# karthik86248/BANG-Billion-Scale-ANN

Measured on AMD Instinct MI355X. Metric: queries/sec, 10K-query batch; SHAPE-ONLY index, L=152, 201 iterations/query (cap-bound), recall n/a; recall-gated: config.recall_gated_* (structured index, 10-recall@10 >= 0.9). A shape-only batch is heavier per query than real data at recall 0.9, higher is better.
Workload: dtype f32

## Files before the change

bang-billion-scale-ann_amd/csrc/bang_search.hip:

```cpp

#include <hip/hip_runtime.h>
#include <type_traits>
#include <utility>
#include <stdint.h>
#include <stdlib.h>
#include <algorithm>

#include "bang_c.h"
#include "bang_internal.h"
#include "bang_device.h"
#include "bang_worklist.h"

struct SearchArgs;
template <class T>
__device__ __forceinline__ T karg_at(size_t off) {
  const char __attribute__((address_space(4)))* ka = (const char __attribute__((address_space(4)))*)__builtin_amdgcn_kernarg_segment_ptr();
  asm volatile("" : "+s"(ka));
  return *(const T __attribute__((address_space(4)))*)(ka + off);
}
__device__ __forceinline__ uint64_t scalar_load_u64(uint64_t tab, uint32_t idx) {
  uint64_t v;
  const uint64_t a = tab + 8ull * idx;
  const uint64_t at = ((uint64_t)uni((uint32_t)(a >> 32)) << 32) | uni((uint32_t)a);
  asm volatile("s_load_dwordx2 %0, %1, 0x0\n\ts_waitcnt lgkmcnt(0)" : "=s"(v) : "s"(at) : "memory");
  return v;
}
#define KARG(field) karg_at<decltype(bang_search_params::field)>(offsetof(SearchArgs, p) + offsetof(bang_search_params, field))
#define KARGP(type, field) ((type GAS*)(uintptr_t)KARG(field))

struct IterArgs {
  const uint8_t* d_codes; uint32_t n_nodes, prio;
  uint32_t* d_cand_ids; const uint8_t* d_graph; uint64_t entry_len;
  uint32_t vec_bytes, row_layout, n_rows_hbm, n_slices;
  const uint32_t* d_rows_hbm; const uint64_t* d_row_slices;
  uint32_t slice_rows, summ_iters;
  uint32_t* d_bloom; uint32_t cap_iter, pad1;
};
enum { IA_CODES = 0, IA_N_NODES = 2, IA_PRIO = 3, IA_CAND_IDS = 4, IA_GRAPH = 6, IA_ENTRY_LEN = 8, IA_VEC_BYTES = 10, IA_ROW_LAYOUT = 11, IA_N_ROWS_HBM = 12,
       IA_N_SLICES = 13, IA_ROWS_HBM = 14, IA_ROW_SLICES = 16, IA_SLICE_ROWS = 18, IA_SUMM_ITERS = 19, IA_BLOOM = 20, IA_CAP_ITER = 22, IA_DWORDS = 24 };
static_assert(sizeof(IterArgs) == 4 * IA_DWORDS && offsetof(IterArgs, d_cand_ids) == 4 * IA_CAND_IDS && offsetof(IterArgs, vec_bytes) == 4 * IA_VEC_BYTES &&
              offsetof(IterArgs, d_rows_hbm) == 4 * IA_ROWS_HBM && offsetof(IterArgs, slice_rows) == 4 * IA_SLICE_ROWS && offsetof(IterArgs, d_bloom) == 4 * IA_BLOOM && offsetof(IterArgs, cap_iter) == 4 * IA_CAP_ITER,
              "IterArgs dword map");
struct SearchArgs {
  bang_search_params p;
  IterArgs iter __attribute__((aligned(16)));
  uint32_t lds_piv_floats;
  uint32_t wave_words;
  uint32_t wl_words;
  uint32_t nctx;
  uint32_t gs;
};

__host__ __device__ constexpr bool search_coop(int ndw, bool host_paced) { return ndw >= 12 && (!host_paced || ndw >= 16); }
__host__ __device__ constexpr bool search_has_spec(int ndw) { return ndw == 18 || ndw == 19; }
__host__ __device__ constexpr int search_maxt(int ndw, bool host_paced);
__host__ __device__ constexpr uint32_t search_scratch_words(int ndw, bool host_paced);

__host__ __device__ inline uint32_t search_wl_words(uint32_t L) { return (2u * L + (L + 3u) / 4u + 3u) & ~3u; }
__host__ __device__ inline uint32_t search_wave_words(uint32_t L, uint32_t nctx, int ndw, bool host_paced) {
  return nctx * search_wl_words(L) + search_scratch_words(ndw, host_paced) + (nctx == 2 ? 32u : 0u);
}

template <int SLOTS>
__device__ __forceinline__ void filter_commit(uint32_t* tbl, int lane, bool& pa, uint32_t ia, uint32_t ba, uint32_t wa, bool& pb,
                                              uint32_t ib, uint32_t bb, uint32_t wb, bool& st_a, uint32_t& out_a, bool& st_b,
                                              uint32_t& out_b) {
  const uint32_t tag_a = (ia << 7) | ((uint32_t)lane << 1), tag_b = (ib << 7) | ((uint32_t)lane << 1) | 1u;
#pragma unroll
  for (int r = 0; r < 3; ++r) {
    if (__ballot(pa || pb) == 0) break;
    const uint32_t mul = r == 0 ? 0x9E37u : r == 1 ? 0x85EBu : 0xC2B3u;
    const uint32_t sa = ((ia * mul) >> 9) & (uint32_t)(SLOTS - 1), sb = ((ib * mul) >> 9) & (uint32_t)(SLOTS - 1);
    if (pa) tbl[sa] = tag_a;
    if (pb) tbl[sb] = tag_b;
    wave_sync();
    const uint32_t ra = tbl[sa], rb = tbl[sb];
    const bool own_a = pa && ra == tag_a, own_b = pb && rb == tag_b;
    const bool same_a = pa && !own_a && (ra >> 7) == ia, same_b = pb && !own_b && (rb >> 7) == ib;
    wave_sync();
    uint32_t va = ba, vb = bb;
    if (__ballot(same_a || same_b)) {
      if (own_a) tbl[sa] = ba;
      if (own_b) tbl[sb] = bb;
      wave_sync();
      if (same_a) (void)__hip_atomic_fetch_or(&tbl[sa], ba, __ATOMIC_RELAXED, __HIP_MEMORY_SCOPE_WAVEFRONT);
      if (same_b) (void)__hip_atomic_fetch_or(&tbl[sb], bb, __ATOMIC_RELAXED, __HIP_MEMORY_SCOPE_WAVEFRONT);
      wave_sync();
      if (own_a) va = tbl[sa];
      if (own_b) vb = tbl[sb];
      wave_sync();
    }
    if (own_a && (wa | va) != wa) { st_a = true; out_a = wa | va; }
    if (own_b && (wb | vb) != wb) { st_b = true; out_b = wb | vb; }
    pa = pa && !(own_a || same_a);
    pb = pb && !(own_b || same_b);
  }
}

#ifndef BANG_FILTER_SUMMARY
#define BANG_FILTER_SUMMARY 1
#endif
template <int SUMM_REGS>
struct FilterSummary {
  uint32_t s[SUMM_REGS];
  __device__ __forceinline__ void clear() {
#pragma unroll
    for (int r = 0; r < SUMM_REGS; ++r) s[r] = 0u;
  }
  static __device__ __forceinline__ uint32_t pos_of(uint32_t w) { const uint32_t p = w >> 6; return p >= 32u * SUMM_REGS ? p - 32u * SUMM_REGS : p; }
  __device__ __forceinline__ bool test(uint32_t w) const {
    const uint32_t p = pos_of(w);
    const int src = (int)((w & 63u) << 2);
    uint32_t v = 0;
#pragma unroll
    for (int r = 0; r < SUMM_REGS; ++r) {
      const uint32_t t = (uint32_t)__builtin_amdgcn_ds_bpermute(src, (int)s[r]);
      v = ((p >> 5) == (uint32_t)r) ? t : v;
    }
    return ((v >> (p & 31u)) & 1u) != 0u;
  }
  template <int RP>
  __device__ __forceinline__ void set(uint32_t* tbl , int lane, bool ha, uint32_t wa, bool hb, uint32_t wb,
                                      bool hc, uint32_t wc0, uint32_t wc1) {
    const uint32_t pa = pos_of(wa), pb = pos_of(wb), pc0 = pos_of(wc0), pc1 = pos_of(wc1);
#pragma unroll
    for (int pass = 0; pass < (SUMM_REGS + RP - 1) / RP; ++pass) {
      if (RP == 2 ? 2 * pass >= SUMM_REGS : 4 * pass >= SUMM_REGS) break;
      const bool ia = ha && (pa >> 5) / RP == (uint32_t)pass, ib = hb && (pb >> 5) / RP == (uint32_t)pass;
      const bool ic0 = hc && (pc0 >> 5) / RP == (uint32_t)pass, ic1 = hc && (pc1 >> 5) / RP == (uint32_t)pass;
      if (__ballot(ia || ib || ic0 || ic1) == 0) continue;
      if (RP == 2) *(uint2*)(tbl + 2 * lane) = make_uint2(0u, 0u);
      else *(uint4*)(tbl + 4 * lane) = make_uint4(0u, 0u, 0u, 0u);
      wave_sync();
      if (ia) (void)__hip_atomic_fetch_or(&tbl[(wa & 63u) * RP + ((pa >> 5) % RP)], 1u << (pa & 31u), __ATOMIC_RELAXED, __HIP_MEMORY_SCOPE_WAVEFRONT);
      if (ib) (void)__hip_atomic_fetch_or(&tbl[(wb & 63u) * RP + ((pb >> 5) % RP)], 1u << (pb & 31u), __ATOMIC_RELAXED, __HIP_MEMORY_SCOPE_WAVEFRONT);
      if (ic0) (void)__hip_atomic_fetch_or(&tbl[(wc0 & 63u) * RP + ((pc0 >> 5) % RP)], 1u << (pc0 & 31u), __ATOMIC_RELAXED, __HIP_MEMORY_SCOPE_WAVEFRONT);
      if (ic1) (void)__hip_atomic_fetch_or(&tbl[(wc1 & 63u) * RP + ((pc1 >> 5) % RP)], 1u << (pc1 & 31u), __ATOMIC_RELAXED, __HIP_MEMORY_SCOPE_WAVEFRONT);
      wave_sync();
      if (RP == 2) {
        const uint2 v = *(const uint2*)(tbl + 2 * lane);
        s[2 * pass] |= v.x;
        if (2 * pass + 1 < SUMM_REGS) s[2 * pass + 1] |= v.y;
      } else {
        const uint4 v = *(const uint4*)(tbl + 4 * lane);
        s[4 * pass] |= v.x;
        if (4 * pass + 1 < SUMM_REGS) s[4 * pass + 1] |= v.y;
        if (4 * pass + 2 < SUMM_REGS) s[4 * pass + 2] |= v.z;
        if (4 * pass + 3 < SUMM_REGS) s[4 * pass + 3] |= v.w;
      }
      wave_sync();
    }
  }
};

__device__ __forceinline__ void group_barrier(uint32_t* bar, uint32_t n, int lane) {
  asm volatile("s_waitcnt lgkmcnt(0)" ::: "memory");
  if (n > 1 && lane == 0) {
    const uint32_t gen = __hip_atomic_load(&bar[1], __ATOMIC_RELAXED, __HIP_MEMORY_SCOPE_WORKGROUP);
    const uint32_t arrived = __hip_atomic_fetch_add(&bar[0], 1u, __ATOMIC_RELAXED, __HIP_MEMORY_SCOPE_WORKGROUP) + 1u;
    if (arrived == n) {
      __hip_atomic_store(&bar[0], 0u, __ATOMIC_RELAXED, __HIP_MEMORY_SCOPE_WORKGROUP);
      asm volatile("s_waitcnt lgkmcnt(0)" ::: "memory");
      __hip_atomic_store(&bar[1], gen + 1u, __ATOMIC_RELAXED, __HIP_MEMORY_SCOPE_WORKGROUP);
    } else {
      while (__hip_atomic_load(&bar[1], __ATOMIC_RELAXED, __HIP_MEMORY_SCOPE_WORKGROUP) == gen) __builtin_amdgcn_s_sleep(1);
    }
  }
  asm volatile("s_waitcnt lgkmcnt(0)" ::: "memory");
  wave_sync();
}

#define SRCH_GO_STOP 0xFFFFFFFFu
#define SRCH_FIN 0xFFFFFFFFu
#define SRCH_CTX_WORDS 16u

#ifndef BANG_LONG_MAXT
#define BANG_LONG_MAXT 768
#endif

__host__ __device__ constexpr int search_maxt(int ndw, bool host_paced) { return (search_coop(ndw, host_paced) && ndw >= 16) ? (host_paced ? 768 : BANG_LONG_MAXT) : 1024; }
__host__ __device__ constexpr uint32_t search_scratch_words(int ndw, bool host_paced) {
  return search_coop(ndw, host_paced) ? ((ndw >= 16 && search_maxt(ndw, host_paced) >= 1024) ? 144u : 256u) : 144u;
}

template <int PSZ, int NDW, bool ALIGNED, int NHI, bool HOST, bool SPEC>
__global__ __launch_bounds__(search_maxt(NDW, HOST)) void search_kernel(const SearchArgs a) {
  extern __shared__ __attribute__((aligned(16))) float lds[];
  const bang_search_params& p = a.p;
  float* piv_lds = lds;
  {
    const float4* src = (const float4*)p.d_pivots_packed;
    float4* dst = (float4*)piv_lds;
    const uint32_t n4 = a.lds_piv_floats >> 2;
    for (uint32_t i0 = threadIdx.x; i0 < n4; i0 += blockDim.x * 8) {
      float4 v[8];
#pragma unroll
      for (int j = 0; j < 8; ++j) {
        const uint32_t i = i0 + (uint32_t)j * blockDim.x;
        v[j] = src[i < n4 ? i : n4 - 1];
      }
#pragma unroll
      for (int j = 0; j < 8; ++j) {
        const uint32_t i = i0 + (uint32_t)j * blockDim.x;
        if (i < n4) dst[i] = v[j];
      }
    }
  }
  const int lane0 = lane_id();
  int lane = lane0;
  const uint32_t wave = uni(threadIdx.x >> 6);
  const uint32_t nwaves = blockDim.x >> 6;
  uint32_t iav;
  {
    const char __attribute__((address_space(4)))* ka = (const char __attribute__((address_space(4)))*)__builtin_amdgcn_kernarg_segment_ptr();
    iav = ((const uint32_t __attribute__((address_space(4)))*)(ka + offsetof(SearchArgs, iter)))[lane0 < IA_DWORDS ? lane0 : 0];
  }
#define IA_FRESH() asm volatile("" : "+v"(iav))
#define IA32(k) ((uint32_t)__builtin_amdgcn_readlane((int)iav, (k)))
#define IA64(k) (((uint64_t)IA32((k) + 1) << 32) | (uint64_t)IA32(k))
#define IAPTR(type, k) ((type GAS*)IA64(k))
  const uint32_t nctx = HOST ? a.nctx : 1u;
  const uint32_t L = p.L, medoid = p.medoid;
  const unsigned long long go_timeout = p.go_timeout_ticks ? p.go_timeout_ticks : BANG_KERNEL_GO_TIMEOUT_TICKS;
  uint32_t* wbase = (uint32_t*)(lds + a.lds_piv_floats) + (size_t)wave * a.wave_words;
  uint32_t* scratch = wbase + (size_t)nctx * a.wl_words;
  uint32_t* park = scratch + search_scratch_words(NDW, HOST);
  const uint32_t gs = HOST ? a.gs : nwaves;
  const uint32_t grp_in_wg = HOST ? wave / gs : 0u;
  const uint32_t gw0 = grp_in_wg * gs;
  const uint32_t gsize = (nwaves - gw0) < gs ? (nwaves - gw0) : gs;
  const uint32_t gslot = wave - gw0;
  const uint32_t ngrp = HOST ? (nwaves + gs - 1) / gs : 1u;
  uint32_t* wg_lds = (uint32_t*)(lds + a.lds_piv_floats) + (size_t)nwaves * a.wave_words + (size_t)grp_in_wg * 128;
  if (HOST && gslot == 0) { wg_lds[lane] = 0u; wg_lds[64 + lane] = 0u; }
  if (HOST && nctx == 2 && lane < (int)(2 * SRCH_CTX_WORDS)) park[lane] = 0u;
  __syncthreads();
  if (p.d_ktime && threadIdx.x == 0) p.d_ktime[2 * blockIdx.x] = __builtin_amdgcn_s_memrealtime();

  float* sd = (float*)scratch;
  uint32_t* ti = scratch;
  float* td = (float*)(scratch + 72);
  uint32_t* sc = scratch + 72;
  uint32_t* tbl = scratch;
  const uint32_t total_waves = gridDim.x * nwaves;
  const uint32_t gw = blockIdx.x * nwaves + wave;
  const uint32_t cand_stride = L + BANG_EXTRA_ITERS;
  constexpr int SB = (NDW >= 18) ? 6 : 0;
  constexpr bool EARLY_ROWS = !HOST;
  constexpr bool COOP = search_coop(NDW, HOST);
  constexpr uint32_t SCR = search_scratch_words(NDW, HOST);
  static_assert(!SPEC || !HOST, "the speculative row request belongs to the self-paced form");

  const uint32_t code_stride = p.code_stride ? p.code_stride : p.m;

  bool active = false, exhausted = false;
  uint32_t q = 0, iter = 0, w_n = 0, cc = 0, mark = 0, evals = 0, fetched = 0;
  uint32_t cnt_in = 0, x0 = 0, x1 = 0;
  bool have_row = false;
  bool self_row = false;
  WlHead head;
  head.found = false; head.idx = 0; head.id = 0; head.d = 0.0f; head.tail = 0.0f;
  constexpr int QW = NDW * 4 * PSZ;
  constexpr bool QC16 = !HOST && ((NDW == 18 && NHI != 0) || NDW == 19);
  constexpr int NV = QC16 ? (QW + 15) / 16 : (QW + 63) / 64;
  typedef typename std::conditional<QC16, QcRow16<NV>, QcRegs<NV>>::type Qc;
  Qc qc;
#pragma unroll
  for (int r = 0; r < NV; ++r) qc.v[r] = 0.0f;
  auto load_qc = [&](uint32_t qq) {
    const float* src = p.d_qc + (size_t)qq * QW;
#pragma unroll
    for (int r = 0; r < NV; ++r) {
      const uint32_t i = QC16 ? (uint32_t)r * 16u + ((uint32_t)lane & 15u) : (uint32_t)r * 64u + (uint32_t)lane;
      qc.v[r] = src[i < (uint32_t)QW ? i : 0u];
    }
  };
  constexpr bool SUMM = (BANG_FILTER_SUMMARY != 0) && (!HOST || search_maxt(NDW, HOST) < 1024);
  FilterSummary<6> summ;
  summ.clear();
  uint32_t probes_skipped = 0;
  uint32_t started = 0;
  uint32_t dead_mask = 0;
  uint32_t rounds0 = 0, rounds1 = 0;
  uint32_t tick = 0;

  unsigned long long pf_poll = 0, pf_front = 0, pf_pub = 0, pf_back = 0, pf_n = 0, pf_t = 0;
  const bool prof = HOST && p.d_prof != nullptr && wave == 0;
#define PF_STAMP(acc) do { if (prof) { const unsigned long long t_ = __builtin_amdgcn_s_memrealtime(); acc += t_ - pf_t; pf_t = t_; } } while (0)
  if (prof) pf_t = __builtin_amdgcn_s_memrealtime();

#ifdef BANG_SEARCH_PHASE_PROF
  unsigned long long ph_acc[12] = {0, 0, 0, 0, 0, 0, 0, 0, 0, 0, 0, 0}, ph_t = __builtin_amdgcn_s_memrealtime(), ph_n = 0;
#define PH(k) do { if (wave == 0) { const unsigned long long t_ = __builtin_amdgcn_s_memrealtime(); ph_acc[k] += t_ - ph_t; ph_t = t_; } } while (0)
#else
#define PH(k) do {} while (0)
#endif

#define LANE_FRESH() do { if (BANG_LONG_MAXT >= 1024) { lane = lane0; asm volatile("" : "+v"(lane)); } } while (0)
  for (uint32_t half = 0;; ++half) {
    LANE_FRESH();
    const uint32_t c = HOST ? (nctx == 2 ? (half & 1u) : 0u) : 0u;
    if (HOST) {
      if (dead_mask == (nctx == 2 ? 3u : 1u)) break;
      if ((dead_mask >> c) & 1u) continue;
    }
    const uint32_t round = HOST ? (c ? rounds1 : rounds0) + 1u : 0u;
    const uint32_t grp = HOST ? (blockIdx.x * ngrp + grp_in_wg) * nctx + c : 0u;
    WaveLds s;
    s.wd = (float*)(wbase + (size_t)c * a.wl_words); s.wi = wbase + (size_t)c * a.wl_words + L; s.wv = (uint8_t*)(wbase + (size_t)c * a.wl_words + 2 * L);
    s.sd = sd; s.ti = ti; s.td = td;
    if (HOST) {
      if (nctx == 2) {
        const uint32_t* pk = park + c * SRCH_CTX_WORDS;
        active = uni(pk[0]) != 0u; q = uni(pk[1]); iter = uni(pk[2]); w_n = uni(pk[3]); cc = uni(pk[4]); mark = uni(pk[5]);
        evals = uni(pk[6]); fetched = uni(pk[7]);
        have_row = uni(pk[8]) != 0u;
        head.found = uni(pk[9]) != 0u; head.idx = uni(pk[10]); head.id = uni(pk[11]);
        head.d = __uint_as_float(uni(pk[12])); head.tail = __uint_as_float(uni(pk[13]));
        if (active) load_qc(q);
      }
      if (round > 1) {
        if (gslot == 0 && lane == 0) {
          const uint32_t* go = p.d_ctl + (size_t)grp * 16;
          uint32_t v = __hip_atomic_load(go, __ATOMIC_RELAXED, __HIP_MEMORY_SCOPE_SYSTEM);
          const unsigned long long t0 = __builtin_amdgcn_s_memrealtime();
          while (v < round - 1u) {
            __builtin_amdgcn_s_sleep(4);
            v = __hip_atomic_load(go, __ATOMIC_RELAXED, __HIP_MEMORY_SCOPE_SYSTEM);
            if (__builtin_amdgcn_s_memrealtime() - t0 > go_timeout) {
              v = SRCH_GO_STOP;
              if (p.d_abort) *p.d_abort = 1u;
              break;
            }
          }
          wg_lds[0] = v;
          __builtin_amdgcn_fence(__ATOMIC_ACQUIRE, "agent");
          asm volatile("s_waitcnt vmcnt(0)" ::: "memory");
        }
        group_barrier(wg_lds + 120, gsize, lane);
        PF_STAMP(pf_poll);
        if (wg_lds[0] == SRCH_GO_STOP) break;
        if (active && have_row && !self_row) {
          const uint32_t cw = p.d_ctl[(size_t)grp * 16 + 1 + (gslot >> 2)];
          cnt_in = (cw >> (8 * (gslot & 3u))) & 0xFFu;
          x0 = p.d_rows[((size_t)grp * 16 + gslot) * 64 + lane];
        }
      }
    }

    if (!active && !exhausted) {
      if (!((started >> c) & 1u)) q = c * total_waves + gw;
      else {
        uint32_t t = 0;
        if (lane == 0) t = __hip_atomic_fetch_add(KARGP(uint32_t, d_next_query), 1u, __ATOMIC_RELAXED, __HIP_MEMORY_SCOPE_AGENT);
        q = nctx * total_waves + uni(t);
      }
      started |= 1u << c;
      if (q < KARG(Q)) {
        active = true;
        w_n = 0; cc = 1; mark = 0x01010101u;
        evals = 0; fetched = 0; iter = 1;
        if (SUMM) { summ.clear(); probes_skipped = 0; }
        if (lane == 0) KARGP(uint32_t, d_cand_ids)[(size_t)q * cand_stride] = medoid;
        load_qc(q);
        { const uint32_t GAS* seed = KARGP(const uint32_t, d_seed); cnt_in = seed[0]; x0 = seed[1 + lane]; x1 = seed[65]; }
        have_row = true;
        self_row = false;
      } else exhausted = true;
    }
    if (!HOST && !active) break;

    uint32_t n = 0, sid0 = 0, sid1 = 0, parent = 0;
    constexpr bool SET_LATE = !HOST;
    bool sl_a = false, sl_b = false;
    uint32_t sl_ua = 0, sl_ub = 0;
    float d0 = BIG_DIST, d1 = BIG_DIST;
    bool found = false;
    const bool first = (iter == 1);
    if (active) {
      uint32_t ci = have_row ? uni(cnt_in) : 0u;
      if (((!HOST && p.row_layout) || (HOST && self_row)) && !first && have_row)
        ci = (uint32_t)__popcll(__ballot(x0 != 0xFFFFFFFFu));
      PH(0);
      {
        const uint32_t cap = p.R + (first ? 1u : 0u);
        if (ci > cap) ci = cap;
      }
      IA_FRESH();
      const uint32_t prio_m = HOST ? 0u : IA32(IA_PRIO);
      const bool prio = (prio_m & 1u) != 0u;
      if (prio) __builtin_amdgcn_s_setprio(3);
      uint32_t GAS* bloom = IAPTR(uint32_t, IA_BLOOM) + (size_t)q * BANG_BF_WORDS;
      const uint32_t n_nodes = HOST ? 0u : IA32(IA_N_NODES);
      if (!HOST && n_nodes != 0u) {
        if (__ballot((uint32_t)lane < ci && x0 >= n_nodes) != 0ull) {
          if (lane == 0 && KARG(d_abort)) *KARGP(uint32_t, d_abort) = 2u;
          ci = 0;
        }
      }
      fetched += ci;
      const bool v0 = (uint32_t)lane < ci;
      const bool v1 = ci > 64;
      const uint32_t h0a = hash1(x0), h0b = hash2(x0);
      uint32_t h1a = 0, h1b = 0, w0a = 0, w0b = 0, w1a = 0, w1b = 0;
      bool la = v0, lb = v0;
      const bool summ_on = SUMM && (HOST || iter <= IA32(IA_SUMM_ITERS));
      if (SUMM && summ_on) {
        la = summ.test(h0a >> 5) && v0;
        lb = summ.test(h0b >> 5) && v0;
        probes_skipped += (uint32_t)__popcll(__ballot(v0 && !la)) + (uint32_t)__popcll(__ballot(v0 && !lb));
      }
      if (la) w0a = ld_bypass_l1(&bloom[h0a >> 5]);
      if (lb) w0b = ld_bypass_l1(&bloom[h0b >> 5]);
      if (v1) {
        h1a = hash1(x1); h1b = hash2(x1);
        if (lane == 0) { w1a = ld_bypass_l1(&bloom[h1a >> 5]); w1b = ld_bypass_l1(&bloom[h1b >> 5]); }
      }
      PqRow<NDW, ALIGNED> row;
      CoopFetch<NDW, ALIGNED> cf;
      const uint8_t GAS* d_codes = IAPTR(const uint8_t, IA_CODES);
      if (SPEC && COOP) cf.issue(d_codes, code_stride, x0, ci < 64u ? ci : 64u, lane);
      else if (SPEC && v0) pq_row_load(row, d_codes, code_stride, x0);
      if (SPEC) asm volatile("" ::: "memory");
      if (prio) __builtin_amdgcn_s_setprio(0);
      const bool pass0 = v0 && !(((w0a >> (h0a & 31)) & 1u) && ((w0b >> (h0b & 31)) & 1u));
      const bool pass1 = v1 && (lane == 0) && !(((w1a >> (h1a & 31)) & 1u) && ((w1b >> (h1b & 31)) & 1u));
      const uint64_t m0 = __ballot(pass0);
      const uint64_t m1 = __ballot(pass1);
      const uint32_t n0 = (uint32_t)__popcll(m0);
      n = n0 + (uint32_t)__popcll(m1);
      PH(1);
      if (pass0) sc[lanes_below(m0)] = x0;
      if (pass1) sc[n0] = x1;
      wave_sync();
      if ((uint32_t)lane < n) sid0 = sc[lane];
      if (lane == 0 && n > 64) sid1 = sc[64];
      wave_sync();
      evals += n;
      PH(2);

      if (!SPEC && EARLY_ROWS) {
        if (COOP) cf.issue(d_codes, code_stride, sid0, n < 64u ? n : 64u, lane);
        else if ((uint32_t)lane < n) pq_row_load(row, d_codes, code_stride, sid0);
      }

      bool pa = pass0, pb = pass0, st_a = false, st_b = false;
      uint32_t sv_a = 0, sv_b = 0;
      filter_commit<SCR >= 256 ? 256 : 128>(tbl, lane, pa, h0a >> 5, 1u << (h0a & 31), w0a, pb, h0b >> 5, 1u << (h0b & 31), w0b, st_a, sv_a, st_b, sv_b);
      if (SUMM && summ_on) {
        if (SET_LATE && !first) { sl_a = pass0 && !la; sl_b = pass0 && !lb; sl_ua = h0a >> 5; sl_ub = h0b >> 5; }
        else summ.template set<SCR >= 256 ? 4 : 2>(tbl, lane, pass0 && !la, h0a >> 5, pass0 && !lb, h0b >> 5, pass1, h1a >> 5, h1b >> 5);
      }
      auto filter_stores = [&]() {
        asm volatile("" ::: "memory");
        if (st_a) bloom[h0a >> 5] = sv_a;
        if (st_b) bloom[h0b >> 5] = sv_b;
        const uint64_t left = __ballot(pa || pb || pass1);
        if (left) {
          asm volatile("s_waitcnt vmcnt(0)" ::: "memory");
          if (pa) (void)__hip_atomic_fetch_or(&bloom[h0a >> 5], 1u << (h0a & 31), __ATOMIC_RELAXED, __HIP_MEMORY_SCOPE_AGENT);
          if (pb) (void)__hip_atomic_fetch_or(&bloom[h0b >> 5], 1u << (h0b & 31), __ATOMIC_RELAXED, __HIP_MEMORY_SCOPE_AGENT);
          if (pass1) {
            (void)__hip_atomic_fetch_or(&bloom[h1a >> 5], 1u << (h1a & 31), __ATOMIC_RELAXED, __HIP_MEMORY_SCOPE_AGENT);
            (void)__hip_atomic_fetch_or(&bloom[h1b >> 5], 1u << (h1b & 31), __ATOMIC_RELAXED, __HIP_MEMORY_SCOPE_AGENT);
          }
        }
      };
      if (!EARLY_ROWS) filter_stores();

      PH(3);
      LANE_FRESH();
      {
        if (COOP && !EARLY_ROWS) cf.issue(d_codes, code_stride, sid0, n < 64u ? n : 64u, lane);
        if (COOP) cf.template collect<(int)SCR>(row, scratch, code_stride, SPEC ? x0 : sid0, lane);
        if (EARLY_ROWS) {
          if (!COOP) {
#pragma unroll
            for (int i = 0; i < PqRow<NDW, ALIGNED>::NX4 * 4; ++i) asm volatile("" : "+v"(row.w[i]));
          }
          filter_stores();
        }
        if (QC16) {
          const float dd = pq_row_reduce_pipe<PSZ, NDW, ALIGNED, NHI>(row, piv_lds, qc);
          if (SPEC) {
            if ((m0 >> lane) & 1ull) sc[lanes_below(m0)] = __float_as_uint(dd);
            wave_sync();
            if ((uint32_t)lane < n0) d0 = __uint_as_float(sc[lane]);
            wave_sync();
          } else if ((uint32_t)lane < n) d0 = dd;
          if (n > 64) {
            PqRow<NDW, ALIGNED> r1;
            pq_row_load(r1, d_codes, code_stride, uni(sid1));
            const float d1v = pq_row_reduce<PSZ, NDW, ALIGNED, NHI, SB>(r1, piv_lds, qc);
            if (lane == 0) d1 = d1v;
          }
        } else {
          if (SPEC) {
            float dd = BIG_DIST;
            if (v0) dd = pq_row_reduce_pipe<PSZ, NDW, ALIGNED, NHI>(row, piv_lds, qc);
            if ((m0 >> lane) & 1ull) sc[lanes_below(m0)] = __float_as_uint(dd);
            wave_sync();
            if ((uint32_t)lane < n0) d0 = __uint_as_float(sc[lane]);
            wave_sync();
          } else if ((uint32_t)lane < n) {
            if (!COOP && !EARLY_ROWS) pq_row_load(row, d_codes, code_stride, sid0);
            d0 = !HOST ? pq_row_reduce_pipe<PSZ, NDW, ALIGNED, NHI>(row, piv_lds, qc)
                       : pq_row_reduce<PSZ, NDW, ALIGNED, NHI, SB>(row, piv_lds, qc);
          }
          if (n > 64) {
            if (lane == 0) {
              PqRow<NDW, ALIGNED> r1;
              pq_row_load(r1, d_codes, code_stride, sid1);
              d1 = pq_row_reduce<PSZ, NDW, ALIGNED, NHI, SB>(r1, piv_lds, qc);
            }
          }
        }
      }

      if (prio_m & 2u) __builtin_amdgcn_s_setprio(3);
      LANE_FRESH();
      const bool elig = (uint32_t)lane < n && sid0 != medoid && d0 < BIG_DIST;
      PH(4);
      uint32_t khi = elig ? __float_as_uint(d0) : 0xFFFFFFFFu, klo = (uint32_t)lane;
      wave_min_key(khi, klo);
      uint32_t bi = (khi != 0xFFFFFFFFu) ? klo : 0xFFFFu;
      float bd = (khi != 0xFFFFFFFFu) ? __uint_as_float(khi) : BIG_DIST;
      uint32_t bid = (uint32_t)__builtin_amdgcn_readlane((int)sid0, (int)(klo & 63u));
      if (n > 64) {
        const float e_d = __shfl(d1, 0);
        const uint32_t e_id = (uint32_t)__shfl((int)sid1, 0);
        if (e_id != medoid && e_d < BIG_DIST && (bi == 0xFFFFu || e_d < bd)) { bd = e_d; bi = 64; bid = e_id; }
      }
      const bool have_best = (bi != 0xFFFFu);
      if (!have_best) bd = BIG_DIST;
      bool from_best = false;
      if (first) {
        if (have_best) { found = true; parent = bid; from_best = true; }
      } else {
        if (head.found) {
          found = true;
          if (bd < head.d) { parent = bid; from_best = true; }
          else { parent = head.id; if (lane == 0) s.wv[head.idx] = 1; }
        } else if (w_n > 0) {
          if (bd < head.tail) { found = true; parent = bid; from_best = true; }
        }
      }
      parent = uni(parent);
      if (found) {
        if (from_best) mark = parent;
        ++cc;
      }
    }
    IA_FRESH();
    const uint32_t cap_iter = IA32(IA_CAP_ITER);
    const bool want_row = active && found && iter < cap_iter;
    PH(5);

    if (!HOST) {
      if (want_row) {
        const uint8_t GAS* gbase = IAPTR(const uint8_t, IA_GRAPH);
        if (IA32(IA_ROW_LAYOUT)) {
          const uint32_t GAS* hb = nullptr;
          const uint32_t nsl = IA32(IA_N_SLICES);
          if (nsl > 1u) {
            const uint32_t sl = parent / IA32(IA_SLICE_ROWS);
            if (sl < nsl) hb = (const uint32_t GAS*)scalar_load_u64(IA64(IA_ROW_SLICES), sl);
          } else if (parent < IA32(IA_N_ROWS_HBM)) hb = IAPTR(const uint32_t, IA_ROWS_HBM);
          if (hb) x0 = hb[(uint64_t)parent * 64u + lane];
          else x0 = __builtin_nontemporal_load((const uint32_t GAS*)gbase + (uint64_t)parent * 64u + lane);
          cnt_in = 64u;
        } else {
          const uint32_t GAS* nrow = (const uint32_t GAS*)(gbase + (uint64_t)parent * IA64(IA_ENTRY_LEN) + IA32(IA_VEC_BYTES));
          cnt_in = nrow[0];
          x0 = nrow[1 + lane];
        }
      }
    } else {
      uint32_t* cnt_act = wg_lds + 1 + (tick % 3u);
      self_row = false;
      if (nctx == 1u && want_row && !p.ship_vectors) {
        if (parent < IA32(IA_N_ROWS_HBM)) { self_row = true; x0 = (IAPTR(const uint32_t, IA_ROWS_HBM))[(uint64_t)parent * 64u + lane]; cnt_in = 64u; }
      }
      if (lane == 0) {
        const bool tell = active && found && (want_row || p.ship_vectors);
        wg_lds[4 + 48 * c + gslot] = tell ? (self_row ? BANG_IDLE_PARENT : parent) : BANG_NO_PARENT;
        wg_lds[20 + 48 * c + gslot] = q | (want_row ? 0x80000000u : 0u);
        wg_lds[36 + 48 * c + gslot] = cc - 1u;
        if (active) (void)__hip_atomic_fetch_add(cnt_act, 1u, __ATOMIC_RELAXED, __HIP_MEMORY_SCOPE_WORKGROUP);
      }
      group_barrier(wg_lds + 120, gsize, lane);
      PF_STAMP(pf_front);
      const bool grp_alive = (*cnt_act != 0u);
      if (gslot == 0) {
        if (grp_alive) {
          if ((uint32_t)lane < gsize) {
            __hip_atomic_store(&p.h_parents[(size_t)grp * 16 + lane], wg_lds[4 + 48 * c + lane], __ATOMIC_RELAXED, __HIP_MEMORY_SCOPE_SYSTEM);
            if (p.ship_vectors) {
              __hip_atomic_store(&p.h_pub_q[(size_t)grp * 16 + lane], wg_lds[20 + 48 * c + lane], __ATOMIC_RELAXED, __HIP_MEMORY_SCOPE_SYSTEM);
              __hip_atomic_store(&p.h_pub_c[(size_t)grp * 16 + lane], wg_lds[36 + 48 * c + lane], __ATOMIC_RELAXED, __HIP_MEMORY_SCOPE_SYSTEM);
            }
          }
          asm volatile("s_waitcnt vmcnt(0)" ::: "memory");
        }
        if (lane == 0) {
          __hip_atomic_store(p.h_done + (size_t)grp * 16, grp_alive ? round : SRCH_FIN, __ATOMIC_RELAXED, __HIP_MEMORY_SCOPE_SYSTEM);
          wg_lds[1 + ((tick + 2u) % 3u)] = 0u;
        }
      }
      ++tick;
      PF_STAMP(pf_pub);
      if (prof) ++pf_n;
      if (!grp_alive) { dead_mask |= 1u << c; continue; }
      if (c) rounds1 = round; else rounds0 = round;
    }

    PH(8);
    if (!HOST && (IA32(IA_PRIO) & 2u) != 0u) __builtin_amdgcn_s_setprio(0);
    if (active && found && lane == 0) IAPTR(uint32_t, IA_CAND_IDS)[(size_t)q * cand_stride + cc - 1u] = parent;
    if (active) {
      LANE_FRESH();
      if (n > 0 && iter < cap_iter) {
        w_n = sort_and_merge(s, n, d0, sid0, d1, sid1, iter, w_n, L, medoid, mark, head.tail, lane);
      }
      PH(6);
#ifdef BANG_SEARCH_PHASE_PROF
      if (wave == 0) ++ph_n;
#endif

      if ((!found && n == 0) || iter == cap_iter) {
        if (lane == 0) {
          KARGP(uint32_t, d_cand_cnt)[q] = cc;
          uint32_t GAS* qstats = KARGP(uint32_t, d_qstats);
          uint32_t GAS* qiters = KARGP(uint32_t, d_qiters);
          uint32_t GAS* qskip = KARGP(uint32_t, d_qskip);
          if (qstats) { qstats[(size_t)q * 2] = evals; qstats[(size_t)q * 2 + 1] = fetched; }
          if (qiters) qiters[q] = iter;
          if (qskip) qskip[q] = probes_skipped;
        }
        if (!HOST) {
          RerankArgs8 rr;
          rr.queries = (const uint8_t GAS*)KARG(rr_queries);
          if (rr.queries) {
            rr.vec_base = (const uint8_t GAS*)KARG(rr_vec_base); rr.vec_stride = KARG(rr_vec_stride); rr.ids_out = (uint64_t GAS*)KARG(rr_ids_out); rr.dists_out = (float GAS*)KARG(rr_dists_out);
            rr.D = KARG(rr_D); rr.k = KARG(rr_k); rr.q0 = KARG(rr_q0); rr.Q_total = KARG(rr_Q_total);
            rr.cand = KARGP(const uint32_t, d_cand_ids) + (size_t)q * cand_stride;
            const uint32_t nc = cc < cand_stride ? cc : cand_stride;
            const uint32_t rdt = KARG(rr_dtype);
            if (rdt == BANG_F32) wave_rerank_f32<4>(rr, q, nc, wbase, lane);
            else if (rdt == BANG_I8) wave_rerank8<true>(rr, q, nc, wbase, lane);
            else wave_rerank8<false>(rr, q, nc, wbase, lane);
          }
        }
        active = false;
      } else {
        ++iter;
        have_row = found;
        head = worklist_head(s, w_n, lane);
        PH(9);
        if (HOST && !self_row) { cnt_in = 0; x0 = 0; }
        if (SUMM && SET_LATE) summ.template set<SCR >= 256 ? 4 : 2>(tbl, lane, sl_a, sl_ua, sl_b, sl_ub, false, 0u, 0u);
        PH(10);
      }
    }
    if (HOST && nctx == 2) {
      uint32_t* pk = park + c * SRCH_CTX_WORDS;
      if (lane == 0) {
        pk[0] = active ? 1u : 0u; pk[1] = q; pk[2] = iter; pk[3] = w_n; pk[4] = cc; pk[5] = mark; pk[6] = evals; pk[7] = fetched;
        pk[8] = have_row ? 1u : 0u;
        pk[9] = head.found ? 1u : 0u; pk[10] = head.idx; pk[11] = head.id; pk[12] = __float_as_uint(head.d); pk[13] = __float_as_uint(head.tail);
      }
      wave_sync();
    }
    PF_STAMP(pf_back);
  }
  if (prof && lane == 0) {
    unsigned long long* o = p.d_prof + (size_t)blockIdx.x * 16;
    o[0] = pf_poll; o[1] = pf_front; o[2] = pf_pub; o[3] = pf_back; o[4] = pf_n;
  }
#undef PF_STAMP
#ifdef BANG_SEARCH_PHASE_PROF
  if (p.d_prof && wave == 0 && lane == 0) {
    unsigned long long* o = p.d_prof + (size_t)blockIdx.x * 16 + 8;
    for (int k = 0; k < 7; ++k) o[k] = ph_acc[k];
    o[7] = ph_n;
    if (!HOST) { unsigned long long* x = p.d_prof + (size_t)blockIdx.x * 16; x[0] = ph_acc[8]; x[1] = ph_acc[9]; x[2] = ph_acc[10]; }
  }
#endif
#undef PH
  if (KARG(d_ktime)) {
    __syncthreads();
    if (threadIdx.x == 0) KARG(d_ktime)[2 * blockIdx.x + 1] = __builtin_amdgcn_s_memrealtime();
  }
}

template <int PSZ, int NDW, bool ALIGNED, int NHI, bool HOST, bool SPEC>
static int launch_inst(const SearchArgs& a, dim3 grid, dim3 block, size_t lds, hipStream_t st) {
  static bool attr_done[BANG_MAX_DEVICES] = {false};
  const int dev = current_device();
  if (!attr_done[dev]) {
    HIP_TRY(hipFuncSetAttribute((const void*)search_kernel<PSZ, NDW, ALIGNED, NHI, HOST, SPEC>, hipFuncAttributeMaxDynamicSharedMemorySize,
                                160 * 1024));
    attr_done[dev] = true;
  }
  hipLaunchKernelGGL((search_kernel<PSZ, NDW, ALIGNED, NHI, HOST, SPEC>), grid, block, lds, st, a);
  HIP_TRY(hipGetLastError());
  return BANG_OK;
}

#ifndef BANG_SEARCH_PART
#define BANG_SEARCH_PART 0
#endif
constexpr bool search_in_part1(int ndw, bool aligned, bool host_paced) { return ndw >= 24 || (ndw == 19 && !aligned) || (host_paced && ndw >= 16); }
extern "C" int bang_search_launch_part1(const SearchArgs* a, uint32_t grid, uint32_t block, size_t lds, void* stream);

template <int PSZ, int NDW, bool ALIGNED, int NHI, bool HOST, bool SPEC>
static int launch_part(const SearchArgs& a, dim3 grid, dim3 block, size_t lds, hipStream_t st) {
  if constexpr (search_in_part1(NDW, ALIGNED, HOST) == (BANG_SEARCH_PART == 1)) return launch_inst<PSZ, NDW, ALIGNED, NHI, HOST, SPEC>(a, grid, block, lds, st);
#if BANG_SEARCH_PART == 0
  return bang_search_launch_part1(&a, grid.x, block.x, lds, (void*)st);
#else
  bang_set_error("search-kernel instance psz=%u mp=%u is not part of this translation unit", a.p.psz, a.p.mp);
  return BANG_ERR_UNSUPPORTED;
#endif
}

template <int PSZ, int NDW, bool ALIGNED, int NHI>
static int launch_hd(const SearchArgs& a, dim3 grid, dim3 block, size_t lds, hipStream_t st) {
  if constexpr (search_has_spec(NDW)) {
    if (a.p.d_graph && a.p.spec_rows == 1u) return launch_part<PSZ, NDW, ALIGNED, NHI, false, true>(a, grid, block, lds, st);
  }
  return a.p.d_graph ? launch_part<PSZ, NDW, ALIGNED, NHI, false, false>(a, grid, block, lds, st)
                     : launch_part<PSZ, NDW, ALIGNED, NHI, true, false>(a, grid, block, lds, st);
}

template <int PSZ, int NDW>
static int launch_al(const SearchArgs& a, dim3 grid, dim3 block, size_t lds, hipStream_t st) {
  const bool al = ((a.p.code_stride ? a.p.code_stride : a.p.m) % 4u) == 0;
  if (a.p.pq_nhi) {
    constexpr int NHI = (PSZ == 2 && NDW == 18) ? 58 : (PSZ == 2 && NDW == 19) ? 22 : 0;
    if constexpr (NHI != 0) {
      if ((int)a.p.pq_nhi == NHI) return al ? launch_hd<PSZ, NDW, true, NHI>(a, grid, block, lds, st) : launch_hd<PSZ, NDW, false, NHI>(a, grid, block, lds, st);
    }
    bang_set_error("no search-kernel instance for the exact-size pivot table psz=%u mp=%u nhi=%u", a.p.psz, a.p.mp, a.p.pq_nhi);
    return BANG_ERR_UNSUPPORTED;
  }
  return al ? launch_hd<PSZ, NDW, true, 0>(a, grid, block, lds, st) : launch_hd<PSZ, NDW, false, 0>(a, grid, block, lds, st);
}

static int search_dispatch(const SearchArgs& a, dim3 grid, dim3 block, size_t lds, hipStream_t st) {
  const bang_search_params* p = &a.p;
  const uint32_t key = p->psz * 100u + p->mp / 4u;
  switch (key) {
#ifndef BANG_DEV_ONLY_218
    case 108: return launch_al<1, 8>(a, grid, block, lds, st);
    case 116: return launch_al<1, 16>(a, grid, block, lds, st);
    case 124: return launch_al<1, 24>(a, grid, block, lds, st);
    case 132: return launch_al<1, 32>(a, grid, block, lds, st);
    case 208: return launch_al<2, 8>(a, grid, block, lds, st);
    case 216: return launch_al<2, 16>(a, grid, block, lds, st);
    case 219: return launch_al<2, 19>(a, grid, block, lds, st);
#endif
    case 218: return launch_al<2, 18>(a, grid, block, lds, st);
#ifndef BANG_DEV_ONLY_218
    case 404: return launch_al<4, 4>(a, grid, block, lds, st);
    case 408: return launch_al<4, 8>(a, grid, block, lds, st);
    case 802: return launch_al<8, 2>(a, grid, block, lds, st);
    case 804: return launch_al<8, 4>(a, grid, block, lds, st);
#endif
    default: bang_set_error("no search-kernel instance for psz=%u mp=%u", p->psz, p->mp); return BANG_ERR_UNSUPPORTED;
  }
}

#if BANG_SEARCH_PART == 1
extern "C" int bang_search_launch_part1(const SearchArgs* a, uint32_t grid, uint32_t block, size_t lds, void* stream) {
  return search_dispatch(*a, dim3(grid), dim3(block), lds, (hipStream_t)stream);
}
#else

#define SRCH_WG_SHARED_BYTES 2048u
#define SRCH_DEFAULT_GROUP_WAVES 8u

static uint32_t waves_that_fit(uint32_t psz, uint32_t mp, uint32_t nhi, uint32_t L, uint32_t nctx, bool host_paced) {
  const size_t piv_bytes = (size_t)pivot_table_floats(psz, mp, nhi) * 4u;
  const size_t per_wave = (size_t)search_wave_words(L, nctx, (int)(mp / 4u), host_paced) * 4u;
  const size_t cap = (size_t)160 * 1024 - (host_paced ? SRCH_WG_SHARED_BYTES : 0u);
  if (piv_bytes + per_wave > cap) return 0;
  const size_t w = (cap - piv_bytes) / per_wave;
  const size_t most = (size_t)search_maxt((int)(mp / 4u), host_paced) / WAVE;
  return (uint32_t)(w > most ? most : w);
}

extern "C" int bang_search_can_rerank(int dtype, uint32_t D, uint64_t vec_stride, uint32_t dim_adjust) {
  const uint32_t G = D >> 4;
  if (dim_adjust != 0 || (vec_stride & 3u) != 0 || D > 256) return 0;
  if (dtype == BANG_F32) return D >= 4 && (D & 3u) == 0;
  return (dtype == BANG_U8 || dtype == BANG_I8) && D >= 16 && (D & 15u) == 0 && (G & (G - 1u)) == 0;
}

extern "C" int bang_search_supported(uint32_t psz, uint32_t mp, uint32_t nhi, uint32_t L) {
  if (psz == 0 || L == 0 || L > BANG_MAX_L) return 0;
  return (int)waves_that_fit(psz, mp, nhi, L, 1, false);
}

extern "C" int bang_search_geometry(uint32_t psz, uint32_t mp, uint32_t nhi, uint32_t L, uint32_t Q, uint32_t max_wgs,
                                    uint32_t max_waves, int host_paced, uint32_t* workgroups, uint32_t* waves_out, uint32_t* nctx_io,
                                    uint32_t* group_waves_io) {
  if (!workgroups || !waves_out || !nctx_io || !group_waves_io || Q == 0) return BANG_ERR_ARG;
  if (psz == 0 || L == 0 || L > BANG_MAX_L) { bang_set_error("bad pq layout / L"); return BANG_ERR_ARG; }
  uint32_t nctx = *nctx_io;
  if (!host_paced) nctx = 1;
  else if (nctx == 0) nctx = 1;
  else if (nctx > 2) nctx = 2;
  if (host_paced && search_maxt((int)(mp / 4u), true) < 1024) nctx = 1;
  uint32_t waves = waves_that_fit(psz, mp, nhi, L, nctx, host_paced != 0);
  if (waves == 0) { bang_set_error("pivot table + one wave's worklist do not fit LDS at L=%u", L); return BANG_ERR_UNSUPPORTED; }
  if (max_waves && max_waves < waves) waves = max_waves;
  const uint32_t cus = (uint32_t)num_cus();
  uint32_t grid_n = Q < cus ? Q : cus;
  if (max_wgs && max_wgs < grid_n) grid_n = max_wgs;
  const uint32_t per_wg = ((Q + grid_n - 1) / grid_n + nctx - 1) / nctx;
  if (per_wg < waves) waves = per_wg;
  else if (!host_paced && per_wg > waves && per_wg <= 2 * waves) waves = (per_wg + 1) / 2;
  uint32_t gs = *group_waves_io ? *group_waves_io : SRCH_DEFAULT_GROUP_WAVES;
  if (gs > 16) gs = 16;
  if (gs < 4) gs = 4;
  if (gs > waves) gs = waves;
  *workgroups = grid_n;
  *waves_out = waves;
  *nctx_io = nctx;
  *group_waves_io = host_paced ? gs : waves;
  return BANG_OK;
}

extern "C" int bang_k_search(const bang_search_params* p, void* stream) {
  if (!p) return BANG_ERR_ARG;
  if (p->Q == 0) return BANG_OK;
  if (p->R == 0 || p->R > BANG_MAX_R || p->L == 0 || p->L > BANG_MAX_L || p->m == 0) { bang_set_error("bad R/L/m"); return BANG_ERR_ARG; }
  if (p->psz == 0 || p->mp < p->m || (p->mp & 3u)) { bang_set_error("the search kernel needs the LDS-resident pivot layout"); return BANG_ERR_UNSUPPORTED; }
  if (!p->d_codes || !p->d_pivots_packed || !p->d_qc || !p->d_seed || !p->d_bloom || !p->d_cand_ids || !p->d_cand_cnt ||
      !p->d_next_query) { bang_set_error("null buffer"); return BANG_ERR_ARG; }
  if (!p->d_graph && (!p->d_rows || !p->d_ctl || !p->h_done || !p->h_parents || (p->ship_vectors && (!p->h_pub_q || !p->h_pub_c)))) {
    bang_set_error("host-paced search kernel: null pacing buffer"); return BANG_ERR_ARG;
  }
  if (p->pq_nhi && (p->psz != 2 || p->pq_nhi > p->mp)) { bang_set_error("bad pq_nhi"); return BANG_ERR_ARG; }
  if (p->cap_iter == 0 || p->cap_iter > p->L + BANG_EXTRA_ITERS - 1) { bang_set_error("bad iteration cap"); return BANG_ERR_ARG; }
  if (p->rr_queries) {
    if (!p->d_graph) { bang_set_error("the fused re-rank belongs to the self-paced form"); return BANG_ERR_ARG; }
    if (!p->rr_vec_base || !p->rr_ids_out || !p->rr_dists_out || p->rr_k == 0 || p->rr_Q_total < p->rr_q0 + p->Q ||
        !bang_search_can_rerank((int)p->rr_dtype, p->rr_D, p->rr_vec_stride, 0) || (((uintptr_t)p->rr_vec_base) & 3u) || (((uintptr_t)p->rr_queries) & 3u)) {
      bang_set_error("fused re-rank: bad arguments / unsupported vector layout"); return BANG_ERR_ARG;
    }
  }
  SearchArgs a;
  a.p = *p;
  a.lds_piv_floats = pivot_table_floats(p->psz, p->mp, p->pq_nhi);
  __builtin_memset(&a.iter, 0, sizeof(a.iter));
  a.iter.d_codes = p->d_codes; a.iter.n_nodes = p->n_nodes; a.iter.d_cand_ids = p->d_cand_ids; a.iter.d_graph = p->d_graph; a.iter.entry_len = p->entry_len;
  a.iter.vec_bytes = p->vec_bytes; a.iter.row_layout = p->row_layout; a.iter.n_rows_hbm = p->n_rows_hbm; a.iter.n_slices = p->n_slices;
  a.iter.d_rows_hbm = p->d_rows_hbm; a.iter.d_row_slices = p->d_row_slices; a.iter.slice_rows = p->slice_rows;
  a.iter.d_bloom = p->d_bloom; a.iter.cap_iter = p->cap_iter;
  uint32_t grid_n = 0, waves = 0, nctx = p->nctx, gs = p->group_waves;
  const int rc = bang_search_geometry(p->psz, p->mp, p->pq_nhi, p->L, p->Q, p->max_wgs, p->max_waves, p->d_graph ? 0 : 1, &grid_n, &waves, &nctx, &gs);
  if (rc != BANG_OK) return rc;
  a.nctx = nctx;
  a.gs = gs;
  const bool light = (p->Q + grid_n - 1) / grid_n <= 5u;
  if (a.p.summ_iters == 0u) a.p.summ_iters = light ? 1u : 0xFFFFFFFFu;
  a.iter.summ_iters = a.p.summ_iters;
  { const char* e = getenv("BANG_SEARCH_PRIO"); a.iter.prio = (e && e[0] >= '0' && e[0] <= '3') ? (e[0] == '1' ? 3u : e[0] == '3' ? 1u : (uint32_t)(e[0] - '0')) : (((p->Q + grid_n - 1) / grid_n <= 10u) ? 3u : 0u); }
  const bool spec_auto = p->row_layout != 0u || (p->Q + grid_n - 1) / grid_n <= 8u;
  a.p.spec_rows = (search_has_spec((int)(p->mp / 4u)) && p->d_graph && (p->spec_rows == 1u || (p->spec_rows == 0u && spec_auto))) ? 1u : 2u;
  a.wl_words = search_wl_words(p->L);
  a.wave_words = search_wave_words(p->L, nctx, (int)(p->mp / 4u), p->d_graph == nullptr);
  const size_t lds = (size_t)a.lds_piv_floats * 4 + (size_t)waves * a.wave_words * 4 + (p->d_graph ? 0u : SRCH_WG_SHARED_BYTES);
  const dim3 grid(grid_n), block(waves * WAVE);
  hipStream_t st = (hipStream_t)stream;
  return search_dispatch(a, grid, block, lds, st);
}
#endif
```

Baseline: 1.241 million.

## Reuse per-wave bloom filter slots across queries and store filter words directly

```diff
diff --git a/bang-billion-scale-ann_amd/csrc/bang_search.hip b/bang-billion-scale-ann_amd/csrc/bang_search.hip
--- a/bang-billion-scale-ann_amd/csrc/bang_search.hip
+++ b/bang-billion-scale-ann_amd/csrc/bang_search.hip
@@ -34,12 +34,14 @@
   uint32_t vec_bytes, row_layout, n_rows_hbm, n_slices;
   const uint32_t* d_rows_hbm; const uint64_t* d_row_slices;
   uint32_t slice_rows, summ_iters;
-  uint32_t* d_bloom; uint32_t cap_iter, pad1;
+  uint32_t* d_bloom; uint32_t cap_iter, slot_filter;
 };
 enum { IA_CODES = 0, IA_N_NODES = 2, IA_PRIO = 3, IA_CAND_IDS = 4, IA_GRAPH = 6, IA_ENTRY_LEN = 8, IA_VEC_BYTES = 10, IA_ROW_LAYOUT = 11, IA_N_ROWS_HBM = 12,
-       IA_N_SLICES = 13, IA_ROWS_HBM = 14, IA_ROW_SLICES = 16, IA_SLICE_ROWS = 18, IA_SUMM_ITERS = 19, IA_BLOOM = 20, IA_CAP_ITER = 22, IA_DWORDS = 24 };
+       IA_N_SLICES = 13, IA_ROWS_HBM = 14, IA_ROW_SLICES = 16, IA_SLICE_ROWS = 18, IA_SUMM_ITERS = 19, IA_BLOOM = 20, IA_CAP_ITER = 22, IA_SLOT = 23,
+       IA_DWORDS = 24 };
 static_assert(sizeof(IterArgs) == 4 * IA_DWORDS && offsetof(IterArgs, d_cand_ids) == 4 * IA_CAND_IDS && offsetof(IterArgs, vec_bytes) == 4 * IA_VEC_BYTES &&
-              offsetof(IterArgs, d_rows_hbm) == 4 * IA_ROWS_HBM && offsetof(IterArgs, slice_rows) == 4 * IA_SLICE_ROWS && offsetof(IterArgs, d_bloom) == 4 * IA_BLOOM && offsetof(IterArgs, cap_iter) == 4 * IA_CAP_ITER,
+              offsetof(IterArgs, d_rows_hbm) == 4 * IA_ROWS_HBM && offsetof(IterArgs, slice_rows) == 4 * IA_SLICE_ROWS && offsetof(IterArgs, d_bloom) == 4 * IA_BLOOM && offsetof(IterArgs, cap_iter) == 4 * IA_CAP_ITER &&
+              offsetof(IterArgs, slot_filter) == 4 * IA_SLOT,
               "IterArgs dword map");
 struct SearchArgs {
   bang_search_params p;
@@ -364,6 +366,22 @@
         if (lane == 0) KARGP(uint32_t, d_cand_ids)[(size_t)q * cand_stride] = medoid;
         load_qc(q);
         { const uint32_t GAS* seed = KARGP(const uint32_t, d_seed); cnt_in = seed[0]; x0 = seed[1 + lane]; x1 = seed[65]; }
+        if (!HOST) {
+          const bool slot = IA32(IA_SLOT) != 0u;
+          if (!slot || q < total_waves) {
+            const uint64_t row = (uint64_t)(uintptr_t)KARG(d_bloom) + (uint64_t)q * (BANG_BF_WORDS * 4u);
+            iav = lane == IA_BLOOM ? (uint32_t)row : lane == IA_BLOOM + 1 ? (uint32_t)(row >> 32) : iav;
+          }
+          if (slot) {
+            static_assert(BANG_BF_WORDS % 4u == 0u && BANG_BF_WORDS - 256u <= 192u * 64u && BANG_BF_WORDS <= 192u * 64u + 256u, "zeroed words vs summary aliases");
+            typedef uint32_t u32x4 __attribute__((ext_vector_type(4)));
+            uint32_t GAS* row = IAPTR(uint32_t, IA_BLOOM);
+            ((u32x4 GAS*)row)[lane] = (u32x4)(0u);
+            ((u32x4 GAS*)row)[(BANG_BF_WORDS - 256u) / 4u + (uint32_t)lane] = (u32x4)(0u);
+            if (lane == 0) { row[hash1(x1) >> 5] = 0u; row[hash2(x1) >> 5] = 0u; }
+            asm volatile("s_waitcnt vmcnt(0)" ::: "memory");
+          }
+        }
         have_row = true;
         self_row = false;
       } else exhausted = true;
@@ -390,7 +408,7 @@
       const uint32_t prio_m = HOST ? 0u : IA32(IA_PRIO);
       const bool prio = (prio_m & 1u) != 0u;
       if (prio) __builtin_amdgcn_s_setprio(3);
-      uint32_t GAS* bloom = IAPTR(uint32_t, IA_BLOOM) + (size_t)q * BANG_BF_WORDS;
+      uint32_t GAS* bloom = IAPTR(uint32_t, IA_BLOOM) + (HOST ? (size_t)q * BANG_BF_WORDS : 0u);
       const uint32_t n_nodes = HOST ? 0u : IA32(IA_N_NODES);
       if (!HOST && n_nodes != 0u) {
         if (__ballot((uint32_t)lane < ci && x0 >= n_nodes) != 0ull) {
@@ -447,14 +465,18 @@
       bool pa = pass0, pb = pass0, st_a = false, st_b = false;
       uint32_t sv_a = 0, sv_b = 0;
       filter_commit<SCR >= 256 ? 256 : 128>(tbl, lane, pa, h0a >> 5, 1u << (h0a & 31), w0a, pb, h0b >> 5, 1u << (h0b & 31), w0b, st_a, sv_a, st_b, sv_b);
+      if (!HOST) {
+        if (pa) sv_a = w0a | (1u << (h0a & 31));
+        if (pb) sv_b = w0b | (1u << (h0b & 31));
+      }
       if (SUMM && summ_on) {
         if (SET_LATE && !first) { sl_a = pass0 && !la; sl_b = pass0 && !lb; sl_ua = h0a >> 5; sl_ub = h0b >> 5; }
         else summ.template set<SCR >= 256 ? 4 : 2>(tbl, lane, pass0 && !la, h0a >> 5, pass0 && !lb, h0b >> 5, pass1, h1a >> 5, h1b >> 5);
       }
       auto filter_stores = [&]() {
         asm volatile("" ::: "memory");
-        if (st_a) bloom[h0a >> 5] = sv_a;
-        if (st_b) bloom[h0b >> 5] = sv_b;
+        if (st_a || (!HOST && pa)) bloom[h0a >> 5] = sv_a;
+        if (st_b || (!HOST && pb)) bloom[h0b >> 5] = sv_b;
         const uint64_t left = __ballot(pa || pb || pass1);
         if (left) {
           asm volatile("s_waitcnt vmcnt(0)" ::: "memory");
@@ -867,6 +889,12 @@
   const bool light = (p->Q + grid_n - 1) / grid_n <= 5u;
   if (a.p.summ_iters == 0u) a.p.summ_iters = light ? 1u : 0xFFFFFFFFu;
   a.iter.summ_iters = a.p.summ_iters;
+  {
+    const char* e = getenv("BANG_SEARCH_SLOT_FILTER");
+    const bool can = BANG_FILTER_SUMMARY != 0 && p->d_graph != nullptr && a.p.summ_iters >= p->cap_iter;
+    const bool want = (e && (e[0] == '0' || e[0] == '1')) ? e[0] == '1' : p->Q > grid_n * waves;
+    a.iter.slot_filter = (can && want) ? 1u : 0u;
+  }
   { const char* e = getenv("BANG_SEARCH_PRIO"); a.iter.prio = (e && e[0] >= '0' && e[0] <= '3') ? (e[0] == '1' ? 3u : e[0] == '3' ? 1u : (uint32_t)(e[0] - '0')) : (((p->Q + grid_n - 1) / grid_n <= 10u) ? 3u : 0u); }
   const bool spec_auto = p->row_layout != 0u || (p->Q + grid_n - 1) / grid_n <= 8u;
   a.p.spec_rows = (search_has_spec((int)(p->mp / 4u)) && p->d_graph && (p->spec_rows == 1u || (p->spec_rows == 0u && spec_auto))) ? 1u : 2u;
```

After: 1.227 million, median of 6. Within noise of the previous version (-1.2%).
